# adamnelsonarcher/BB-OCR

Measured on AMD Instinct MI355X. Metric: book-page images/sec end-to-end (detect+recognize) @1280x960, higher is better.
Workload: dtype fp16

## Files before the change

bb-ocr_amd/csrc/common.h:

```cpp
#pragma once
#include <hip/hip_runtime.h>
#include <stdint.h>
#include <atomic>
#include <string>

typedef __attribute__((ext_vector_type(8))) __bf16 bf16x8;
typedef __attribute__((ext_vector_type(8))) short s16x8;
typedef __attribute__((ext_vector_type(4))) float f32x4;
typedef __attribute__((ext_vector_type(4))) unsigned int u32x4;
typedef __attribute__((ext_vector_type(2))) unsigned int u32x2;

static inline uint16_t f32_to_bf16_host(float f) {
    uint32_t u;
    __builtin_memcpy(&u, &f, 4);
    if ((u & 0x7fffffffu) > 0x7f800000u) return (uint16_t)((u >> 16) | 0x40);
    u += 0x7fffu + ((u >> 16) & 1u);
    return (uint16_t)(u >> 16);
}
static inline float bf16_to_f32_host(uint16_t h) {
    uint32_t u = ((uint32_t)h) << 16;
    float f;
    __builtin_memcpy(&f, &u, 4);
    return f;
}
// ... 5 lines not shown
    __bf16 b = (__bf16)f;
    return __builtin_bit_cast(unsigned short, b);
}
typedef __attribute__((ext_vector_type(2))) __bf16 bf16x2_t;
typedef __attribute__((ext_vector_type(2))) float f32x2_t;
__device__ __forceinline__ unsigned int pack_bf16x2(float lo, float hi) {
    const f32x2_t v = {lo, hi};
    return __builtin_bit_cast(unsigned int, __builtin_convertvector(v, bf16x2_t));
}

typedef __attribute__((ext_vector_type(8))) _Float16 f16x8;
typedef __attribute__((ext_vector_type(2))) _Float16 f16x2_t;
static inline uint16_t f32_to_f16_host(float f) {
    const _Float16 h = (_Float16)f;
    uint16_t u;
    __builtin_memcpy(&u, &h, 2);
    return u;
}
static inline float f16_to_f32_host(uint16_t u) {
    _Float16 h;
    __builtin_memcpy(&h, &u, 2);
    return (float)h;
}
static inline uint16_t f32_to_el_host(int el, float f) { return el ? f32_to_f16_host(f) : f32_to_bf16_host(f); }
static inline float el_to_f32_host(int el, uint16_t u) { return el ? f16_to_f32_host(u) : bf16_to_f32_host(u); }

template <int EL> struct El;
template <> struct El<0> {
    typedef bf16x8 v8;
    static __device__ __forceinline__ f32x4 mfma(v8 a, v8 b, f32x4 c) { return __builtin_amdgcn_mfma_f32_16x16x32_bf16(a, b, c, 0, 0, 0); }
    static __device__ __forceinline__ unsigned int pack2(float lo, float hi) { return pack_bf16x2(lo, hi); }
    static __device__ __forceinline__ f32x2_t unpack2(unsigned int q) { return (f32x2_t){__uint_as_float(q << 16), __uint_as_float(q & 0xffff0000u)}; }
    static __device__ __forceinline__ unsigned short from_f32(float f) { return f32_to_bf16_bits(f); }
    static __device__ __forceinline__ float to_f32(unsigned short h) { return bf16_bits_to_f32(h); }
};
template <> struct El<1> {
    typedef f16x8 v8;
    static __device__ __forceinline__ f32x4 mfma(v8 a, v8 b, f32x4 c) { return __builtin_amdgcn_mfma_f32_16x16x32_f16(a, b, c, 0, 0, 0); }
    static __device__ __forceinline__ unsigned int pack2(float lo, float hi) {
        const f32x2_t v = {lo, hi};
        return __builtin_bit_cast(unsigned int, __builtin_convertvector(v, f16x2_t));
    }
    static __device__ __forceinline__ f32x2_t unpack2(unsigned int q) { return __builtin_convertvector(__builtin_bit_cast(f16x2_t, q), f32x2_t); }
    static __device__ __forceinline__ unsigned short from_f32(float f) { return __builtin_bit_cast(unsigned short, (_Float16)f); }
    static __device__ __forceinline__ float to_f32(unsigned short h) { return (float)__builtin_bit_cast(_Float16, h); }
};
__device__ __forceinline__ s16x8 sm16_key(s16x8 x) { return x ^ ((x >> 15) & (short)0x7fff); }

__device__ __forceinline__ int xcd_remap(int bid, int nblk) {
    const int q = nblk >> 3, r = nblk & 7, x = bid & 7, i = bid >> 3;
    return (x < r ? x * (q + 1) : r * (q + 1) + (x - r) * q) + i;
}

#define HIP_TRY(expr)                                                                      \
    do {                                                                                   \
        hipError_t _e = (expr);                                                            \
        if (_e != hipSuccess) {                                                            \
            throw std::string(#expr) + ": " + hipGetErrorString(_e);                       \
        }                                                                                  \
    } while (0)

static constexpr int kMaxDev = 32;
struct LdsOptIn {
    std::atomic<size_t> hw[kMaxDev];
};
static inline hipError_t lds_opt_in(LdsOptIn& st, const void* fn, size_t smem) {
    int d = 0;
    hipError_t e = hipGetDevice(&d);
    if (e != hipSuccess) return e;
    if (d < 0 || d >= kMaxDev) return hipErrorInvalidDevice;
    size_t cur = st.hw[d].load(std::memory_order_acquire);
    if (smem <= cur) return hipSuccess;
    e = hipFuncSetAttribute(fn, hipFuncAttributeMaxDynamicSharedMemorySize, (int)smem);
    if (e != hipSuccess) return e;
    while (cur < smem && !st.hw[d].compare_exchange_weak(cur, smem, std::memory_order_release)) {}
    return hipSuccess;
}
static inline int device_cus() {
    static std::atomic<int> n[kMaxDev];
    int d = 0;
    if (hipGetDevice(&d) != hipSuccess || d < 0 || d >= kMaxDev) return 256;
    int v = n[d].load(std::memory_order_acquire);
    if (v) return v;
    hipDeviceProp_t prop;
    v = (hipGetDeviceProperties(&prop, d) == hipSuccess && prop.multiProcessorCount > 0) ? prop.multiProcessorCount : 256;
    n[d].store(v, std::memory_order_release);
    return v;
}
```

bb-ocr_amd/csrc/conv_mfma.hip:

```cpp
#include "common.h"
#include "kernels.h"
#include <type_traits>
#include <utility>

__device__ __forceinline__ void lds_dma16(const void* gptr, const void* lds) {
    const unsigned la = (unsigned)(size_t)(const __attribute__((address_space(3))) void*)lds;
    asm volatile("s_mov_b32 m0, %1\n\ts_nop 0\n\tglobal_load_lds_dwordx4 %0, off" ::"v"(gptr), "s"(la) : "memory");
}

template <int EL, int MF, bool ADDUP = false>
__device__ __forceinline__ void conv_epilogue(const ConvArgs& a, f32x4 (&acc)[MF][4], int n, int nt, int oy0, int ox0, int wm, int wn, int fpr,
                                              int lane, int BN, int sub = 1, int sph = 0, int spw = 0) {
    const int g = lane >> 4, pl = lane & 15;
    const int cout0 = nt * BN + wn * 64 + g * 8;
    if (a.tail) {
        const float* tw = a.tail;
        const typename El<EL>::v8 w1f = *(const typename El<EL>::v8*)(a.tail_frag + lane * 8);
        float cb[8], b1r[4], w2a[4], w2b[4];
#pragma unroll
        for (int i = 0; i < 8; ++i) cb[i] = a.bias[(g & 1) * 8 + i];
#pragma unroll
        for (int r = 0; r < 4; ++r) { b1r[r] = tw[4 * g + r]; w2a[r] = tw[16 + 4 * g + r]; w2b[r] = tw[32 + 4 * g + r]; }
        const float b20 = tw[48], b21 = tw[49];
#pragma unroll
        for (int f = 0; f < MF; ++f) {
            const int F = wm * MF + f;
            const int fr = F / fpr, fc = F - fr * fpr;
            const int oy = (oy0 + fr) * sub + sph, ox = (ox0 + fc * 16 + pl) * sub + spw;
            u32x4 bb;
#pragma unroll
            for (int j = 0; j < 2; ++j) {
                const float x0 = fmaxf(acc[f][j][0] + cb[j * 4 + 0], 0.f), x1 = fmaxf(acc[f][j][1] + cb[j * 4 + 1], 0.f);
                const float x2 = fmaxf(acc[f][j][2] + cb[j * 4 + 2], 0.f), x3 = fmaxf(acc[f][j][3] + cb[j * 4 + 3], 0.f);
                bb[2 * j] = g < 2 ? El<EL>::pack2(x0, x1) : 0u;
                bb[2 * j + 1] = g < 2 ? El<EL>::pack2(x2, x3) : 0u;
            }
            const f32x4 d = El<EL>::mfma(w1f, __builtin_bit_cast(typename El<EL>::v8, bb), (f32x4){0.f, 0.f, 0.f, 0.f});
            float p0 = 0.f, p1 = 0.f;
#pragma unroll
            for (int r = 0; r < 4; ++r) {
                const float hv = fmaxf(d[r] + b1r[r], 0.f);
                p0 = fmaf(w2a[r], hv, p0);
                p1 = fmaf(w2b[r], hv, p1);
            }
            p0 += __shfl_xor(p0, 16); p1 += __shfl_xor(p1, 16);
            p0 += __shfl_xor(p0, 32); p1 += __shfl_xor(p1, 32);
            if (g == 0 && oy < a.OH && ox < a.OW) *(float2*)((float*)a.out + ((size_t)(n * a.OH + oy) * a.OW + ox) * 2) = make_float2(p0 + b20, p1 + b21);
        }
        return;
    }
    const bool run0 = cout0 < a.cout_store, run1 = cout0 + 32 < a.cout_store;
    if (!run0) return;
    const float sc = a.acc_scale;
    float bs[16];
#pragma unroll
    for (int h = 0; h < 2; ++h)
#pragma unroll
        for (int q = 0; q < 2; ++q) {
            const f32x4 b4 = *(const f32x4*)(a.bias + cout0 + h * 32 + q * 4);
            bs[h * 8 + q * 4 + 0] = b4[0]; bs[h * 8 + q * 4 + 1] = b4[1]; bs[h * 8 + q * 4 + 2] = b4[2]; bs[h * 8 + q * 4 + 3] = b4[3];
        }
// ... 1493 lines not shown
```

bb-ocr_amd/csrc/ctx.h:

```cpp
#pragma once
#include "../../include/bbocr.h"

#include <algorithm>
#include <atomic>
#include <chrono>
#include <condition_variable>
#include <cmath>
#include <cstring>
#include <functional>
#include <map>
#include <memory>
#include <mutex>
#include <string>
#include <thread>
#include <unordered_map>
#include <vector>

#include "boxpost.h"
#include "hostpool.h"
#include "common.h"
#include "kernels.h"


using clk = std::chrono::steady_clock;
// ... 273 lines not shown
};

struct RecChunk {
    int imgW, T, first, n;
    size_t row0;
};

struct RecPart {
    std::vector<CropDesc> descs;
    std::vector<int> order;
    std::vector<RecChunk> chunks;
    size_t rows = 0, cols = 0;
    bool any_warp = false, any_tall = false;
};

struct RecRun {
    std::vector<int> tiles, seqs, seq_k;
    size_t rows = 0;
    int n_results = 0;
};

struct RecEarly {
    bool active = false;
    int pages = 0;
    std::vector<BoxJob> jobs;
    std::vector<int> box_off;
    size_t a_total = 0, w_total = 0;
    RecPart part;
};

constexpr int REC_GAP = 4;
constexpr int REC_STAGES = 8;

template <typename T> inline T* upload(bbocr_ctx* c, const std::vector<T>& v) {
    void* d = nullptr;
    HIPCHK(hipMalloc(&d, v.size() * sizeof(T)));
    c->owned.push_back(d);
    c->owned_bytes.push_back(v.size() * sizeof(T));
    HIPCHK(hipMemcpy(d, v.data(), v.size() * sizeof(T), hipMemcpyHostToDevice));
    return (T*)d;
}

ConvPlan make_plan(int Cin, int Cout, int KH, int KW, int pad, int dil, int el = 0, int bn = 0);
void upload_plan(bbocr_ctx* c, ConvPlan& p, const std::vector<float>& w, const std::vector<float>& b);
void free_weights(bbocr_ctx* c);
size_t weights_blob_bytes(const bbocr_ctx* c);
void weights_export(bbocr_ctx* c, void* dev_dst, size_t bytes);
void weights_import(bbocr_ctx* c, const void* dev_src, size_t bytes);
void load_craft(bbocr_ctx* c, const TensorMap& tm);
void load_crnn(bbocr_ctx* c, const TensorMap& tm);
ConvArgs conv_args(const ConvPlan& p, const Act& a0, const Act* a1 = nullptr, const Act* addup = nullptr);
hipError_t launch_conv_profiled(bbocr_ctx* c, const ConvPlan& p, ConvArgs a, bool may_decline = false);
void run_conv(bbocr_ctx* c, const ConvPlan& p, const Act& a0, bool relu0, const Act* a1, bool relu1, bool relu_out, void* out, int out_cs, int cout_store, bool out_f32, const Act* addup = nullptr);
void prof_collect(bbocr_ctx* c);
Act conv_act(bbocr_ctx* c, const ConvPlan& p, const Act& a0, bool relu0, const Act* a1, bool relu1, bool relu_out, int store);
Act conv_pool_act(bbocr_ctx* c, const ConvPlan& p, const Act& a0, bool relu0, bool relu_out, int store, int mode, bool pool_relu, Act* full, const RgbSource* rgb = nullptr);
Act pool_act(bbocr_ctx* c, const Act& a, int kh, int kw, int sh, int sw, int ph, int pw, bool relu_in);
void craft_up_stage(bbocr_ctx* c, const ConvPlan& py, const ConvPlan& ps, const Act& y, const Act& skip, uint16_t* z, uint16_t* out);
bool craft_up3b_post(bbocr_ctx* c, const Act& u3a, uint16_t* u3b, uint16_t* z);
bool craft_up4(bbocr_ctx* c, const Act& s1, const uint16_t* z, uint16_t* u4b);
void craft_cls_tail(bbocr_ctx* c, const Act& c2, float* heat);
struct ExactConvRow {
    const char* name;
    ConvPlan bbocr_ctx::* plan;
    bool relu_out;
    int store;
    int pool_mode;
    bool pool_relu;
    bool keep_full;
};
int craft_exact_rows();
const ExactConvRow& craft_exact_row(int row);
Act craft_exact_conv(bbocr_ctx* c, int row, const Act& in, Act* full = nullptr);
Act craft_exact_conv1_1(bbocr_ctx* c, const uint8_t* rgb, int nb, int Himg, int Wimg, int H32, int W32);
Act craft_exact_relu(bbocr_ctx* c, const Act& a);
Act craft_exact_upcat(bbocr_ctx* c, const Act& y, const Act& skip);
Act craft_exact_pool5(bbocr_ctx* c, const Act& s4);
void craft_exact_cls_tail(bbocr_ctx* c, const Act& c3, float* heat);
DetDims det_dims(int H, int W, int canvas, double mag);
void detect_impl(bbocr_ctx* c, const uint8_t* rgb, int B, int H, int W, const bbocr_params& p, float* heat, const std::function<void(int, int)>& after_sub = nullptr);
DetPlan det_plan(bbocr_ctx* c, int B, int H, int W, const bbocr_params& p, bool overlapped);
void det_size(bbocr_ctx* c, size_t arena_bytes, size_t resized_bytes);
void det_run(bbocr_ctx* c, const DetPlan& s, const uint8_t* rgb, float* heat, const std::function<void(int, int)>& after_sub = nullptr);
int ccl_cap_comps(int B, int h, int w);
void ccl_size(bbocr_ctx* c, size_t npx, int cap_comps);
void boxes_impl(bbocr_ctx* c, const float* heat, int B, int h, int w, double ratio, const bbocr_params& p, HostBoxes& hb, hipStream_t st);
bbocr_boxlist* export_boxes(const HostBoxes& hb);
void import_boxes(const bbocr_boxlist* bl, HostBoxes& hb);
bool plan_horizontal(const std::array<int, 4>& box, int img, int H, int W, BoxJob& j);
bool plan_free(const std::array<double, 8>& fq, int img, BoxJob& j);
int rec_mode(const bbocr_ctx* c);
void crop_refit_fw(CropDesc& d);
void rec_layout_scratch(std::vector<BoxJob>& jobs, size_t first, size_t& a_total, size_t& w_total);
bool contrast_lut(const unsigned int* hist, size_t npx, double target, uint8_t* lut);
std::vector<int> crop_contrast_luts(bbocr_ctx* c, const CropDesc* descs_dev, std::vector<CropDesc>& descs, double target, std::vector<uint8_t>& luts);
void rec_launch_crops(bbocr_ctx* c, const GrayPages& g, const RecPart& part, const CropDesc* dd, uint16_t* wide, int stage);
void rec_plan_part(const std::vector<BoxJob>& jobs, const std::vector<int>& sel, int res0, size_t row_base, RecPart& part);
const CropDesc* rec_upload_descs(bbocr_ctx* c, const RecPart& part, DevBuf& desc_buf);
uint16_t* rec_wide_image(bbocr_ctx* c, const RecPart& part);
void crnn_features_wide(bbocr_ctx* c, const RecPart& part, const CropDesc* descs, const uint16_t* wide);
Act crnn_stage_shape(const bbocr_ctx* c, const RecPart& part, int stage);
Act crnn_features_stages(bbocr_ctx* c, const RecPart& part, const CropDesc* descs, Act a, int first, int last);
void rec_add_tables(RecRun& run, const RecPart& part, int tile_seqs);
void crnn_sequence(bbocr_ctx* c, size_t rows, size_t rows_pad, const int* tiles_dev, int ntiles, const int* seqs_dev, int nseq, float* logits);
void crnn_seq_xproj(bbocr_ctx* c, int l, const uint16_t* x, size_t rows_pad, void* xp);
void crnn_seq_lin(bbocr_ctx* c, int l, const uint16_t* h, size_t rows_pad, uint16_t* out);
void crnn_seq_pred(bbocr_ctx* c, const uint16_t* x, size_t rows_pad, float* logits);
void rec_seq_tiles(const bbocr_ctx* c, RecRun& run);
enum { CTC_GREEDY = 0, CTC_BEAM_HOST = 1, CTC_BEAM_DEVICE = 2 };
int ctc_route(int beam_width, int C, const int* seqs, int nseq);
void ctc_size(bbocr_ctx* c, size_t rows, int nseq, int cs, int route);
double ctc_decode(const CtcOut& o, const int* idx, int n, std::vector<int>& text);
void rec_early_begin(bbocr_ctx* c, const GrayPages& g, int pages, int B, const HostBoxes& hb, const bbocr_params& p, RecEarly& e);
void recognize_impl(bbocr_ctx* c, const GrayPages& g, int B, const HostBoxes& hb, const bbocr_params& p, std::vector<BoxJob>& jobs, std::vector<int>& box_off, RecEarly* early = nullptr);
bbocr_result* export_result(int B, const std::vector<BoxJob>& jobs, const std::vector<int>& box_off);
void pp_resize(bbocr_ctx* c, const uint8_t* src, int H, int W, uint8_t* dst, int dh, int dw, bool src_bgr = false);
void pp_gauss(bbocr_ctx* c, const uint8_t* src, int H, int W, uint8_t* dst, double sigma);
const uint8_t* pp_fold_lut(bbocr_ctx* c, size_t n, double contrast, double brightness);
void pp_clahe(bbocr_ctx* c, const uint8_t* src, int H, int W, const uint8_t* d_lut, uint8_t* dst, double clip_limit);
void pp_unsharp(bbocr_ctx* c, const uint8_t* src, int H, int W, uint8_t* dst, uint8_t* tmp1, uint8_t* tmp2, float radius, int percent, int threshold);
void preprocess_chain_impl(bbocr_ctx* c, const uint8_t* bgr, int H, int W, const bbocr_preproc_params& q, uint8_t* out, int dh, int dw);
void gaussian_taps_fixed(int n, double sigma, int* k);

inline HostPool& host_pool(bbocr_ctx* c) {
    if (!c->pool) {
        const int want = c->cfg.host_threads > 0 ? c->cfg.host_threads : std::min(16, host_cpu_share());
        c->pool.reset(new HostPool(std::max(1, std::min(want, 64)) - 1));
    }
    return *c->pool;
}

inline bool other_call_in_flight(bbocr_ctx* c) {
    bbocr_ctx* root = c->root;
    std::lock_guard<std::mutex> lk(root->pool_mu);
    if (root != c && root->slot_busy) return true;
    for (bbocr_ctx* s : root->slots)
        if (s != c && s->slot_busy) return true;
    return false;
}

struct EnqLock {
    std::unique_lock<std::mutex> lk;
    explicit EnqLock(bbocr_ctx* c) : lk(c->root->enq_mu) {}
};
constexpr int kMaxSlots = 2;
bbocr_ctx* slot_create(bbocr_ctx* root);
void slot_destroy(bbocr_ctx* s);
void publish_times(const bbocr_ctx* s);
void dist_release(bbocr_ctx* root);

inline void slot_sync(bbocr_ctx* c, hipStream_t st) {
    if (!c->sync_ev) HIPCHK(hipEventCreateWithFlags(&c->sync_ev, hipEventDisableTiming));
    HIPCHK(hipEventRecord(c->sync_ev, st));
    HIPCHK(hipEventSynchronize(c->sync_ev));
}

inline void prof_release(bbocr_ctx* c, const bbocr_ctx::ProfRec& r) { c->prof_pool.push_back(r.e0); c->prof_pool.push_back(r.e1); }

// ... 116 lines not shown
```

bb-ocr_amd/csrc/detector.cpp:

```cpp
#include "ctx.h"

static hipEvent_t prof_event(bbocr_ctx* c) {
    hipEvent_t e;
    if (!c->prof_pool.empty()) { e = c->prof_pool.back(); c->prof_pool.pop_back(); }
    else HIPCHK(hipEventCreate(&e));
    return e;
}

template <typename F> static hipError_t profiled(bbocr_ctx* c, double flops, F&& launch) {
    if (c->profiling == 0 || (c->profiling == 1 && c->prof_group != 0)) return launch();
    bbocr_ctx::ProfRec r{prof_event(c), prof_event(c), flops, c->prof_group};
    HIPCHK(hipEventRecord(r.e0, c->cur));
    const hipError_t e = launch();
    HIPCHK(hipEventRecord(r.e1, c->cur));
    if (e == hipSuccess) c->prof_recs.push_back(r);
    else prof_release(c, r);
    return e;
}

hipError_t launch_conv_profiled(bbocr_ctx* c, const ConvPlan& p, ConvArgs a, bool may_decline) {
    a.zero = c->zero_page;
    const int OH = a.H + 2 * p.pad_h - (p.KH - 1) * p.dil, OW = a.W + 2 * p.pad_w - (p.KW - 1) * p.dil;
    double flops = 2.0 * a.N * OH * OW * (double)p.Cout * (p.split ? p.Cin / 3 : p.Cin) * p.KH * p.KW;
    if (a.c11_w) flops += 2.0 * a.N * a.H * a.W * 64.0 * 27.0;
    if (a.tail) flops += 2.0 * a.N * OH * OW * (16.0 * 16.0 + 16.0 * 2.0);
    if (a.post_w) flops += 2.0 * a.N * OH * OW * 64.0 * 64.0;
    const hipError_t e = profiled(c, flops, [&] { return launch_conv(p, a, c->cur); });
    if (may_decline && e == hipErrorNotSupported) return e;
    HIPCHK(e);
    return hipSuccess;
}

ConvArgs conv_args(const ConvPlan& p, const Act& a0, const Act* a1, const Act* addup) {
    ConvArgs a{};
    a.in0 = a0.p; a.C0 = a0.C; a.in0_cs = a0.C;
    a.N = a0.N; a.H = a0.H; a.W = a0.W;
    if (p.split) {
        if (a1 || (a0.C & 63)) fail(BBOCR_ERR_INTERNAL, "split-fp16 conv: one pair tensor with a multiple of 32 logical channels expected");
        a.in1 = a0.p; a.C1 = a0.C / 2; a.in1_cs = a0.C;
    } else if (a1) {
        a.in1 = a1->p; a.C1 = a1->C; a.in1_cs = a1->C;
    }
    if (addup) { a.addup = addup->p; a.up_H = a0.H; a.up_W = a0.W; a.up_cs = addup->C; }
    return a;
}

void run_conv(bbocr_ctx* c, const ConvPlan& p, const Act& a0, bool relu0, const Act* a1, bool relu1, bool relu_out, void* out,
                     int out_cs, int cout_store, bool out_f32, const Act* addup) {
    if (c->arena.dry) return;
    ConvArgs a = conv_args(p, a0, a1, addup);
    a.relu_in0 = relu0; a.relu_in1 = p.split ? relu0 : relu1; a.relu_out = relu_out; a.out_f32 = out_f32;
    a.out = out; a.out_cs = out_cs; a.cout_store = cout_store;
    if (p.split && !out_f32) a.split_off = cout_store;
    (void)launch_conv_profiled(c, p, a);
}

void prof_collect(bbocr_ctx* c) {
    bbocr_ctx* root = c->root;
    std::lock_guard<std::mutex> lk(root->pool_mu);
    for (auto& r : c->prof_recs) {
        float ms = 0.f;
        if (hipEventElapsedTime(&ms, r.e0, r.e1) == hipSuccess) {
            root->prof_ms[r.group] += ms;
            root->prof_flops[r.group] += r.flops;
            root->prof_launches[r.group] += 1;
        }
        prof_release(c, r);
    }
    c->prof_recs.clear();
}

static Act arena_act(bbocr_ctx* c, int N, int H, int W, int C) { return Act{c->arena.alloc<uint16_t>((size_t)N * H * W * C), N, H, W, C}; }

Act conv_act(bbocr_ctx* c, const ConvPlan& p, const Act& a0, bool relu0, const Act* a1, bool relu1, bool relu_out, int store) {
    const int OH = a0.H + 2 * p.pad_h - (p.KH - 1) * p.dil, OW = a0.W + 2 * p.pad_w - (p.KW - 1) * p.dil;
    const int cs = p.split ? 2 * store : store;
    Act o = arena_act(c, a0.N, OH, OW, cs);
    run_conv(c, p, a0, relu0, a1, relu1, relu_out, o.p, cs, store, false);
    return o;
}

Act conv_pool_act(bbocr_ctx* c, const ConvPlan& p, const Act& a0, bool relu0, bool relu_out, int store, int mode, bool pool_relu,
                         Act* full, const RgbSource* rgb) {
// ... 387 lines not shown
```

bb-ocr_amd/csrc/kernels.h:

```cpp
#pragma once
#include <hip/hip_runtime.h>
#include <stdint.h>
#include <vector>

struct ConvArgs {
    const uint16_t* in0;
    const uint16_t* in1;
    const uint16_t* wpk;
    const float* bias;
    void* out;
    int C0, C1;
    int in0_cs, in1_cs;
    int N, H, W, OH, OW;
    int KH, KW, pad_h, pad_w, dil;
    int TH, TW, tiles_x, tiles_y, ntiles_n;
    int PH, PW, NP;
    int relu_in0, relu_in1, relu_out, out_f32;
    int out_cs, cout_store;
    int nchunks, ntaps;
    int pool_mode, pool_relu, store_full, pool_cs;
    void* pool_out;
    const uint16_t* aux_w;
    const float* tail;
    const uint16_t* tail_frag;
// ... 80 lines not shown
hipError_t launch_pair_relu(const uint16_t* in, uint16_t* out, size_t npix, int C, hipStream_t s);
hipError_t launch_pair_maxpool3x3s1(const uint16_t* in, uint16_t* out, int N, int H, int W, int C, hipStream_t s);
hipError_t launch_pair_upcat(const uint16_t* y, int yh, int yw, int Cy, const uint16_t* skip, int Cs, uint16_t* out, int N, int H, int W, hipStream_t s);
hipError_t launch_pair_cls_tail(const uint16_t* in , const float* w1 , const float* tail , float* heat,
                                size_t npix, hipStream_t s);

struct CclOut {
    int root, left, top, right, bottom, area, row_off, img;
};
hipError_t launch_ccl(const float* heat, int N, int h, int w, float low_text, float link_thr, double text_thr, int* label, int* stat,
                      int* slot, CclOut* comps, int* rowext, int* counters, int cap_comps, int cap_rows, hipStream_t s);

struct CropDesc {
    int img;
    int sx0, sy0, sw, sh;
    int rw, rh;
    int fw;
    int imgW;
    int slot;
    int warp;
    int warp_off;
    int a_off;
    int lut_off;
    int pad_;
    int rot;
    double Minv[9];
};
struct CropPage {
    long long off;
    long long pitch;
    int H, W;
};
hipError_t launch_crops(const uint8_t* gray, int H, int W, const CropDesc* descs_dev, int first, int count, int imgW, int any_warp,
                        int any_tall, uint8_t* wscratch, uint8_t* scratch, uint8_t* hscratch, const uint8_t* luts, uint16_t* out_bucket,
                        int stage_mask, hipStream_t s, int wide_row_stride = 0, int gap = 0, int mode = 0,
                        const CropPage* pages = nullptr);
enum { REC_BF16 = 0, REC_F16 = 1, REC_SPLIT = 2 };
constexpr float SPLIT_LO_SCALE = 2048.f;
hipError_t launch_crop_hist(const uint8_t* scratch, const CropDesc* descs_dev, int first, int count, unsigned int* hist, hipStream_t s);
hipError_t launch_crnn_conv0(const uint16_t* in, const float* w , const float* b, uint16_t* out, int n, int W, int mode, hipStream_t s,
                             const uint16_t* afrag = nullptr );
void pack_crnn_conv0_mfma(const float* w_tap_major , uint16_t* out , int el);
hipError_t launch_crnn_zero_gaps(uint16_t* t, const CropDesc* descs_dev, int first, int count, int H, int Wl, int C, int shift, hipStream_t s);
hipError_t launch_rowmean3_gather(const uint16_t* in, int Wc, int C, const CropDesc* descs_dev, int first, int count, uint16_t* out, int mode,
                                  hipStream_t s);
hipError_t launch_lstm(const void* xproj, const uint16_t* whh_pk, uint16_t* out, const int* tiles_dev, int ntiles, int mode, float acc_scale,
                       hipStream_t s);
int lstm_tile_seqs(int mode);
size_t lstm_whh_packed_elems();
void pack_lstm_whh8(const float* whh_fwd, const float* whh_bwd, uint16_t* out, int el);
size_t lstm_whh_split_packed_elems();
float pack_lstm_whh_split(const float* whh_fwd, const float* whh_bwd, uint16_t* out);
int lstm8_xproj_channel(int dir, int gate, int unit);
size_t q8_packed_bytes(int N, int K);
void pack_q8_weights(const int8_t* q , int N, int K, int8_t* out);
void pack_q8_whh(const int8_t* q_fwd, const int8_t* q_bwd , int8_t* out );
hipError_t launch_q8_quantize(const void* x, int src_pair, int K, size_t rows, size_t rows_pad, const int* seqs_dev, int nseq, float* rowp, int8_t* a8,
                              uint8_t* codes, float* segp, hipStream_t s);
hipError_t launch_q8_gemm(const int8_t* a8, size_t rows_pad, int K, const int8_t* wpk, int N, const float* rowp, const float* wscale, const float* bias,
                          float* out, int ldo, hipStream_t s);
constexpr int LSTM_Q8_SEQS = 16;
hipError_t launch_lstm_q8(const float* G, const int8_t* whh_pk, const float* whh_scale, const float* bhh, float* out, const int* seqs_dev,
                          const int* tiles_dev, int ntiles, float* c_out, uint8_t* hcodes, float* hparams, hipStream_t s);
struct CtcOut { int len; int cnt; float prod; int pad; };
hipError_t launch_ctc(const float* logits, size_t rows, int C, int cs, const int* seqs_dev, int nseq, int* idx_tmp, float* pmax_tmp,
                      int* out_idx, CtcOut* out, hipStream_t s, const unsigned int* ignore = nullptr, float* probs_out = nullptr);
void ctc_beam_search_host(const float* mat, int T, int C, int cs, int beam_width, std::vector<int>& text);
class HostPool;
void ctc_beam_search_batch(const float* probs, const int* seqs, int nseq, int C, int cs, int beam_width, std::vector<std::vector<int>>& texts,
                           HostPool* pool = nullptr);
constexpr size_t kCtcBeamLdsLimit = 65536;
size_t ctc_beam_lds_bytes(int beam_width, int C, int max_T);
bool ctc_beam_on_device(int beam_width, int C, int max_T);
hipError_t launch_ctc_beam(const float* probs, size_t rows, int C, int cs, const int* seqs_dev, int nseq, int max_T, int beam_width, int* out_text,
                           int* out_len, hipStream_t s);

int pp_resize_tile_rows(int H, int W, int dh, int dw);
hipError_t launch_pp_resize_cubic(const uint8_t* src, int H, int W, uint8_t* dst, int dh, int dw, const int* x0, const double* wx, const long long* nx,
                                  const int* y0, const double* wy, const long long* ny, unsigned long long KX, unsigned long long KY, hipStream_t s, int src_bgr = 0);
hipError_t launch_pp_gauss3(const uint8_t* src, int H, int W, uint8_t* dst, int k0, int k1, int k2, unsigned long long* sum, hipStream_t s);
hipError_t launch_pp_clahe_hist(const uint8_t* src, int H, int W, const uint8_t* lut, int tw, int th, int tx, int ty, unsigned int* hist,
                                hipStream_t s);
hipError_t launch_pp_clahe_apply(const uint8_t* src, int H, int W, const uint8_t* lut, const uint8_t* tile_luts, int tw, int th, int tx, int ty,
                                 uint8_t* dst, hipStream_t s);
hipError_t launch_pp_box_pass(const uint8_t* src, uint8_t* dst, int H, int W, int vertical, int r, unsigned int ww, unsigned int fw, hipStream_t s);
hipError_t launch_pp_fold_lut(const unsigned long long* sum, unsigned long long n, float contrast, float brightness, uint8_t* lut, hipStream_t s);
hipError_t launch_pp_clahe_luts(const unsigned int* hist, int tiles, int clip, float lut_scale, uint8_t* tile_luts, hipStream_t s);
hipError_t launch_pp_lut(const uint8_t* src, uint8_t* dst, const uint8_t* lut, size_t total, hipStream_t s);
bool pp_unsharp_fused_ok(int H, int W, int r, const uint8_t* a, const uint8_t* b, const uint8_t* c);
hipError_t launch_pp_unsharp_fused(const uint8_t* in, uint8_t* tmp, uint8_t* dst, int H, int W, unsigned int ww, unsigned int fw, int percent,
                                   int threshold, hipStream_t s);
hipError_t launch_pp_unsharp(const uint8_t* in, const uint8_t* blur, uint8_t* dst, size_t total, int percent, int threshold, hipStream_t s);

constexpr int AC_BOX = 35, AC_BOX_R = 17, AC_MEAN_C = 10;
constexpr int AC_GAU = 31, AC_GAU_R = 15, AC_GAU_C = 5;
struct AcTaps { int k[AC_GAU]; };
hipError_t launch_ac_gray_blur(const uint8_t* src, int H, int W, size_t pitch, int channels, uint8_t* dst, hipStream_t s);
hipError_t launch_ac_cues(const uint8_t* e, int H, int W, const AcTaps& taps, uint16_t* rbox, uint16_t* rgau, uint8_t* part, uint8_t* grad,
                          unsigned int* hist, int* thr, hipStream_t s);
hipError_t launch_ac_pack(const uint8_t* e, const uint8_t* part, const uint8_t* grad, const int* thr, int H, int W, int WW, uint32_t* bits, hipStream_t s);
hipError_t launch_ac_rect(const uint32_t* src, uint32_t* tmp, uint32_t* dst, int H, int W, int WW, int rx, int ry, int erode, const uint32_t* or_with,
                          hipStream_t s);
hipError_t launch_ac_components(const uint32_t* bits, int H, int W, int WW, int* label, uint8_t* flag, int* count, int cap, int* boxes, hipStream_t s);
hipError_t launch_ac_unpack(const uint32_t* bits, const int* label, int H, int W, int WW, uint8_t* dst, hipStream_t s);

enum : int { PAGE_GRAY = 0, PAGE_BGR = 1, PAGE_RGB = 2, PAGE_YCC4 = 3, PAGE_YCC3 = 4 };
// ... 135 lines not shown
```

bb-ocr_amd/csrc/recognizer.cpp:

```cpp
#include "ctx.h"

void crop_refit_fw(CropDesc& d) {
    const int cw = (int)std::ceil(64 * ((double)d.rw / (double)d.rh));
    d.fw = cw > d.imgW ? d.imgW : cw;
}

static bool plan_sizes(CropDesc& d, int width, int height) {
    double ratio = (double)width / (double)height;
    if (ratio < 1.0) {
        ratio = 1.0 / ratio;
        d.rw = 64; d.rh = (int)(64 * ratio);
    } else {
        d.rw = (int)(64 * ratio); d.rh = 64;
    }
    if ((int)(64 * ratio) == 0) return false;
    d.imgW = (int)std::ceil(std::max(ratio, 1.0)) * 64;
    crop_refit_fw(d);
    return d.rw > 0 && d.rh > 0 && d.fw > 0;
}

bool plan_horizontal(const std::array<int, 4>& box, int img, int H, int W, BoxJob& j) {
    const int x_min = std::max(0, box[0]), x_max = std::min(box[1], W), y_min = std::max(0, box[2]), y_max = std::min(box[3], H);
    const int width = x_max - x_min, height = y_max - y_min;
    if (width <= 0 || height <= 0) return false;
// ... 86 lines not shown
    c->seq_rowp.ensure(rows_pad * 16);
    int8_t* a8 = (int8_t*)c->seq_q8.p;
    float* rowp = (float*)c->seq_rowp.p;
    auto qlinear = [&](const void* x, int pair, int K, const bbocr_ctx::Q8Layer& L, int N, float* out) {
        HIPCHK(launch_q8_quantize(x, pair, K, rows, rows_pad, seqs_dev, nseq, rowp, a8, nullptr, nullptr, c->cur));
        HIPCHK(launch_q8_gemm(a8, rows_pad, K, L.w, N, rowp, L.scale, L.bias, out, N, c->cur));
    };
    const void* cur = c->seq_v.p;
    for (int l = 0; l < 2; ++l) {
        qlinear(cur, l == 0, 256, c->q_ih[l], 2048, (float*)c->seq_xp.p);
        HIPCHK(launch_lstm_q8((const float*)c->seq_xp.p, c->q_hh[l].w, c->q_hh[l].scale, c->q_hh[l].bias, (float*)c->seq_h.p, seqs_dev, tiles_dev, ntiles,
                              nullptr, nullptr, nullptr, c->cur));
        float* dst = (float*)(l == 0 ? c->seq_lin.p : c->seq_v.p);
        qlinear(c->seq_h.p, 0, 512, c->q_lin[l], 256, dst);
        cur = dst;
    }
    qlinear(cur, 0, 256, c->q_pred, 112, logits);
}

void rec_seq_tiles(const bbocr_ctx* c, RecRun& run) {
    if (!rec_quant(c)) return;
    run.tiles.clear();
    const int nseq = (int)(run.seqs.size() / 2);
    for (int s0 = 0; s0 < nseq; s0 += LSTM_Q8_SEQS) {
        const int n = std::min(LSTM_Q8_SEQS, nseq - s0);
        int tmax = 0;
        for (int i = 0; i < n; ++i) tmax = std::max(tmax, run.seqs[2 * (s0 + i) + 1]);
        const int t[4] = {s0, n, tmax, 0};
        run.tiles.insert(run.tiles.end(), t, t + 4);
    }
}

void crnn_sequence(bbocr_ctx* c, size_t rows, size_t rows_pad, const int* tiles_dev, int ntiles, const int* seqs_dev, int nseq, float* logits) {
    c->prof_group = 1;
    c->arena.dry = false;
    if (rec_quant(c)) { crnn_sequence_q8(c, rows, rows_pad, tiles_dev, ntiles, seqs_dev, nseq, logits); return; }
    const bool sp = rec_split(c);
    const int m = rec_mul(c);
    c->seq_xp.ensure(rows_pad * 2048 * (sp ? 4 : 2));
    c->seq_h.ensure(rows_pad * 512 * 2 * m);
    c->seq_lin.ensure(rows_pad * 256 * 2 * m);
    const uint16_t* cur = (const uint16_t*)c->seq_v.p;
    for (int l = 0; l < 2; ++l) {
        crnn_seq_xproj(c, l, cur, rows_pad, c->seq_xp.p);
        HIPCHK(launch_lstm(c->seq_xp.p, c->whh[l], (uint16_t*)c->seq_h.p, tiles_dev, ntiles, rec_mode(c), c->whh_scale[l], c->cur));
        uint16_t* dst = (uint16_t*)(l == 0 ? c->seq_lin.p : c->seq_v.p);
        crnn_seq_lin(c, l, (const uint16_t*)c->seq_h.p, rows_pad, dst);
        cur = dst;
    }
    crnn_seq_pred(c, cur, rows_pad, logits);
}

static Act seq_rows(const bbocr_ctx* c, const uint16_t* p, size_t rows_pad, int C) { return Act{(uint16_t*)p, 1, (int)(rows_pad / 256), 256, C * rec_mul(c)}; }
void crnn_seq_xproj(bbocr_ctx* c, int l, const uint16_t* x, size_t rows_pad, void* xp) {
    run_conv(c, c->xproj[l], seq_rows(c, x, rows_pad, 256), false, nullptr, false, false, xp, 2048, 2048, rec_split(c));
}
void crnn_seq_lin(bbocr_ctx* c, int l, const uint16_t* h, size_t rows_pad, uint16_t* out) {
    run_conv(c, c->lin[l], seq_rows(c, h, rows_pad, 512), false, nullptr, false, false, out, 256 * rec_mul(c), 256, false);
}
void crnn_seq_pred(bbocr_ctx* c, const uint16_t* x, size_t rows_pad, float* logits) {
    run_conv(c, c->pred, seq_rows(c, x, rows_pad, 256), false, nullptr, false, false, logits, 112, 112, true);
}

static size_t rec_max_rows(const bbocr_ctx* c) { return c->cfg.rec_max_cols > 0 ? (size_t)std::max(64, c->cfg.rec_max_cols / 4) : (size_t)1500000; }

void rec_plan_part(const std::vector<BoxJob>& jobs, const std::vector<int>& sel, int res0, size_t row_base, RecPart& part) {
    std::map<int, std::vector<int>> buckets;
    for (size_t k = 0; k < sel.size(); ++k) buckets[jobs[sel[k]].d.imgW].push_back((int)k);
    size_t rows = row_base, cols = 0;
    for (auto& kv : buckets) {
        const int imgW = kv.first, T = imgW / 4 - 1;
        RecChunk ch{imgW, T, (int)part.descs.size(), (int)kv.second.size(), rows};
        for (int i = 0; i < ch.n; ++i) {
            const int k = kv.second[i];
            CropDesc d = jobs[sel[k]].d;
            if (cols > 0x7ff00000u) fail(BBOCR_ERR_OVERFLOW, "recogniser pass wider than 2^31 columns");
            d.slot = (int)cols;
            d.pad_ = (int)(rows + (size_t)i * T);
            cols += (size_t)imgW + REC_GAP;
            part.any_warp |= d.warp != 0;
            part.any_tall |= !(d.fw == d.rw && d.rh == 64);
            part.descs.push_back(d);
            part.order.push_back(res0 + k);
        }
        rows += (size_t)ch.n * T;
        part.chunks.push_back(ch);
    }
    part.rows = rows - row_base;
    part.cols = cols;
}

const CropDesc* rec_upload_descs(bbocr_ctx* c, const RecPart& part, DevBuf& desc_buf) {
    const size_t bytes = part.descs.size() * sizeof(CropDesc);
    desc_buf.ensure(bytes);
    PinBuf& pin = (&desc_buf == &c->crop_desc2) ? c->desc_pin2 : c->desc_pin;
    pin.ensure(bytes);
    memcpy(pin.p, part.descs.data(), bytes);
    HIPCHK(hipMemcpyAsync(desc_buf.p, pin.p, bytes, hipMemcpyHostToDevice, c->stream));
    return (const CropDesc*)desc_buf.p;
}

uint16_t* rec_wide_image(bbocr_ctx* c, const RecPart& part) {
    c->arena.begin(true);
    (void)c->arena.alloc<uint16_t>((size_t)64 * part.cols);
    crnn_features_wide(c, part, nullptr, nullptr);
    c->arena.buf.ensure(c->arena.off);
    c->arena.begin(false);
    return c->arena.alloc<uint16_t>((size_t)64 * part.cols);
// ... 449 lines not shown
```

Before: 975.1.

## Add dedicated weight-stationary persistent kernel for LSTM input projection

Adds a specialized GEMM kernel for the 256->2048 LSTM input projection. Each block keeps its 256-column weight slice in registers and streams 64-row slots of activations through a 4-deep LDS ring filled by direct global-to-LDS DMA, with counted vmcnt waits to overlap loads, MFMA and stores. It replaces the generic conv path when split mode is off and falls back to it otherwise. This trades generality and register pressure for removing repeated weight loads and pipeline overhead.

```diff
diff --git a/bb-ocr_amd/csrc/common.h b/bb-ocr_amd/csrc/common.h
--- a/bb-ocr_amd/csrc/common.h
+++ b/bb-ocr_amd/csrc/common.h
@@ -81,7 +81,12 @@
     return (x < r ? x * (q + 1) : r * (q + 1) + (x - r) * q) + i;
 }
 
-#define HIP_TRY(expr)                                                                      \
+__device__ __forceinline__ void lds_dma16(const void* gptr, const void* lds) {
+    const unsigned la = (unsigned)(size_t)(const __attribute__((address_space(3))) void*)lds;
+    asm volatile("s_mov_b32 m0, %1\n\ts_nop 0\n\tglobal_load_lds_dwordx4 %0, off" ::"v"(gptr), "s"(la) : "memory");
+}
+
+#define HIP_TRY(expr)                                                                     \
     do {                                                                                   \
         hipError_t _e = (expr);                                                            \
         if (_e != hipSuccess) {                                                            \
diff --git a/bb-ocr_amd/csrc/conv_mfma.hip b/bb-ocr_amd/csrc/conv_mfma.hip
--- a/bb-ocr_amd/csrc/conv_mfma.hip
+++ b/bb-ocr_amd/csrc/conv_mfma.hip
@@ -2,11 +2,6 @@
 #include "kernels.h"
 #include <type_traits>
 #include <utility>
-
-__device__ __forceinline__ void lds_dma16(const void* gptr, const void* lds) {
-    const unsigned la = (unsigned)(size_t)(const __attribute__((address_space(3))) void*)lds;
-    asm volatile("s_mov_b32 m0, %1\n\ts_nop 0\n\tglobal_load_lds_dwordx4 %0, off" ::"v"(gptr), "s"(la) : "memory");
-}
 
 template <int EL, int MF, bool ADDUP = false>
 __device__ __forceinline__ void conv_epilogue(const ConvArgs& a, f32x4 (&acc)[MF][4], int n, int nt, int oy0, int ox0, int wm, int wn, int fpr,
diff --git a/bb-ocr_amd/csrc/ctx.h b/bb-ocr_amd/csrc/ctx.h
--- a/bb-ocr_amd/csrc/ctx.h
+++ b/bb-ocr_amd/csrc/ctx.h
@@ -349,6 +349,7 @@
 ConvArgs conv_args(const ConvPlan& p, const Act& a0, const Act* a1 = nullptr, const Act* addup = nullptr);
 hipError_t launch_conv_profiled(bbocr_ctx* c, const ConvPlan& p, ConvArgs a, bool may_decline = false);
 void run_conv(bbocr_ctx* c, const ConvPlan& p, const Act& a0, bool relu0, const Act* a1, bool relu1, bool relu_out, void* out, int out_cs, int cout_store, bool out_f32, const Act* addup = nullptr);
+hipError_t launch_seq_proj_profiled(bbocr_ctx* c, const ConvPlan& p, const uint16_t* x, size_t rows_pad, uint16_t* out);
 void prof_collect(bbocr_ctx* c);
 Act conv_act(bbocr_ctx* c, const ConvPlan& p, const Act& a0, bool relu0, const Act* a1, bool relu1, bool relu_out, int store);
 Act conv_pool_act(bbocr_ctx* c, const ConvPlan& p, const Act& a0, bool relu0, bool relu_out, int store, int mode, bool pool_relu, Act* full, const RgbSource* rgb = nullptr);
@@ -401,6 +402,7 @@
 void rec_add_tables(RecRun& run, const RecPart& part, int tile_seqs);
 void crnn_sequence(bbocr_ctx* c, size_t rows, size_t rows_pad, const int* tiles_dev, int ntiles, const int* seqs_dev, int nseq, float* logits);
 void crnn_seq_xproj(bbocr_ctx* c, int l, const uint16_t* x, size_t rows_pad, void* xp);
+void crnn_seq_xproj_conv(bbocr_ctx* c, int l, const uint16_t* x, size_t rows_pad, void* xp);
 void crnn_seq_lin(bbocr_ctx* c, int l, const uint16_t* h, size_t rows_pad, uint16_t* out);
 void crnn_seq_pred(bbocr_ctx* c, const uint16_t* x, size_t rows_pad, float* logits);
 void rec_seq_tiles(const bbocr_ctx* c, RecRun& run);
diff --git a/bb-ocr_amd/csrc/detector.cpp b/bb-ocr_amd/csrc/detector.cpp
--- a/bb-ocr_amd/csrc/detector.cpp
+++ b/bb-ocr_amd/csrc/detector.cpp
@@ -29,6 +29,13 @@
     if (may_decline && e == hipErrorNotSupported) return e;
     HIPCHK(e);
     return hipSuccess;
+}
+
+hipError_t launch_seq_proj_profiled(bbocr_ctx* c, const ConvPlan& p, const uint16_t* x, size_t rows_pad, uint16_t* out) {
+    const double flops = 2.0 * (double)rows_pad * (double)p.Cout * p.Cin;
+    const hipError_t e = profiled(c, flops, [&] { return launch_seq_proj(p, x, rows_pad, out, c->cur); });
+    if (e != hipErrorNotSupported) HIPCHK(e);
+    return e;
 }
 
 ConvArgs conv_args(const ConvPlan& p, const Act& a0, const Act* a1, const Act* addup) {
diff --git a/bb-ocr_amd/csrc/kernels.h b/bb-ocr_amd/csrc/kernels.h
--- a/bb-ocr_amd/csrc/kernels.h
+++ b/bb-ocr_amd/csrc/kernels.h
@@ -156,6 +156,9 @@
 size_t lstm_whh_split_packed_elems();
 float pack_lstm_whh_split(const float* whh_fwd, const float* whh_bwd, uint16_t* out);
 int lstm8_xproj_channel(int dir, int gate, int unit);
+struct SeqProjPlan { int grid, chunks, ring; long long nslots, chunk_slots; };
+SeqProjPlan seq_proj_plan(size_t rows_pad, int ncu);
+hipError_t launch_seq_proj(const ConvPlan& p, const uint16_t* x, size_t rows_pad, uint16_t* out, hipStream_t s);
 size_t q8_packed_bytes(int N, int K);
 void pack_q8_weights(const int8_t* q , int N, int K, int8_t* out);
 void pack_q8_whh(const int8_t* q_fwd, const int8_t* q_bwd , int8_t* out );
diff --git a/bb-ocr_amd/csrc/recognizer.cpp b/bb-ocr_amd/csrc/recognizer.cpp
--- a/bb-ocr_amd/csrc/recognizer.cpp
+++ b/bb-ocr_amd/csrc/recognizer.cpp
@@ -162,8 +162,15 @@
 }
 
 static Act seq_rows(const bbocr_ctx* c, const uint16_t* p, size_t rows_pad, int C) { return Act{(uint16_t*)p, 1, (int)(rows_pad / 256), 256, C * rec_mul(c)}; }
+void crnn_seq_xproj_conv(bbocr_ctx* c, int l, const uint16_t* x, size_t rows_pad, void* xp) {
+    run_conv(c, c->xproj[l], seq_rows(c, x, rows_pad, 256), false, nullptr, false, false, xp, 2048, 2048, rec_split(c));
+}
 void crnn_seq_xproj(bbocr_ctx* c, int l, const uint16_t* x, size_t rows_pad, void* xp) {
-    run_conv(c, c->xproj[l], seq_rows(c, x, rows_pad, 256), false, nullptr, false, false, xp, 2048, 2048, rec_split(c));
+    if (!rec_split(c)) {
+        if (c->arena.dry) return;
+        if (launch_seq_proj_profiled(c, c->xproj[l], x, rows_pad, (uint16_t*)xp) == hipSuccess) return;
+    }
+    crnn_seq_xproj_conv(c, l, x, rows_pad, xp);
 }
 void crnn_seq_lin(bbocr_ctx* c, int l, const uint16_t* h, size_t rows_pad, uint16_t* out) {
     run_conv(c, c->lin[l], seq_rows(c, h, rows_pad, 512), false, nullptr, false, false, out, 256 * rec_mul(c), 256, false);
diff --git a/bb-ocr_amd/csrc/seq_proj.hip b/bb-ocr_amd/csrc/seq_proj.hip
--- /dev/null
+++ b/bb-ocr_amd/csrc/seq_proj.hip
@@ -0,0 +1,130 @@
+#include "common.h"
+#include "kernels.h"
+
+namespace {
+constexpr int SP_K = 256, SP_N = 2048;
+constexpr int SP_WAVES = 8, SP_COLS = SP_WAVES * 64, SP_CG = SP_N / SP_COLS;
+constexpr int SP_RING = 4, SP_SLOT_ROWS = 64, SP_SLOT = SP_SLOT_ROWS * SP_K * 2;
+constexpr int SP_DMAS = SP_SLOT / 1024 / SP_WAVES;
+constexpr int SP_STORES = (SP_SLOT_ROWS / 16) * 2;
+constexpr size_t SP_LDS = (size_t)SP_RING * SP_SLOT;
+static_assert(SP_DMAS * SP_WAVES * 1024 == SP_SLOT && SP_DMAS == SP_SLOT_ROWS / 16 && SP_WAVES == SP_K / 32, "wave w fetches k-step w of the slot's four 16-row blocks");
+static_assert((SP_RING - 1) * SP_STORES + (SP_RING - 2) * SP_DMAS < 64, "the counted wait must fit vmcnt's 6 bits");
+
+template <int EL>
+__global__ void __launch_bounds__(SP_WAVES * 64, 2) seq_proj_kernel(const uint16_t* __restrict__ x, const uint16_t* __restrict__ wpk, const float* __restrict__ bias,
+                                                                    uint16_t* __restrict__ out, float acc_scale, int nslots, int chunk_slots) {
+    typedef typename El<EL>::v8 v8;
+    extern __shared__ __attribute__((aligned(16))) unsigned char smem[];
+    const int lane = threadIdx.x & 63;
+    const int wave = __builtin_amdgcn_readfirstlane(threadIdx.x >> 6);
+    const int bid = xcd_remap(blockIdx.x, gridDim.x);
+    const int cg = bid % SP_CG, chunk = bid / SP_CG;
+    const int s0 = chunk * chunk_slots;
+    const int n = nslots - s0 < chunk_slots ? nslots - s0 : chunk_slots;
+    if (n <= 0) return;
+    const int nt = cg * 2 + (wave >> 2), wn = wave & 3;
+    const int g = lane >> 4, pl = lane & 15;
+    const int cout0 = nt * 256 + wn * 64 + g * 8;
+
+    typedef const __attribute__((address_space(1))) v8* gfrag_ptr;
+    const gfrag_ptr wg = (gfrag_ptr)((const v8*)wpk + ((size_t)nt * 8 * 16 + wn * 4) * 64 + lane);
+    v8 w[8][4];
+#pragma unroll
+    for (int ks = 0; ks < 8; ++ks)
+#pragma unroll
+        for (int j = 0; j < 4; ++j) w[ks][j] = wg[(ks * 16 + j) * 64];
+    f32x4 bs[4];
+#pragma unroll
+    for (int j = 0; j < 4; ++j) bs[j] = *(const __attribute__((address_space(1))) f32x4*)(bias + cout0 + (j >> 1) * 32 + (j & 1) * 4);
+
+    const uint16_t* src = x + ((size_t)s0 * SP_SLOT_ROWS + (lane >> 2)) * SP_K + wave * 32 + ((lane & 3) ^ (((lane >> 4) & 1) * 2)) * 8;
+    auto issue = [&](int s, int ring) {
+        unsigned char* sb = smem + ring * SP_SLOT + wave * 4096;
+#pragma unroll
+        for (int i = 0; i < SP_DMAS; ++i) lds_dma16(src + ((size_t)s * SP_SLOT_ROWS + i * 16) * SP_K, sb + i * 1024);
+    };
+#pragma unroll
+    for (int i = 0; i < SP_RING - 1; ++i)
+        if (i < n) issue(i, i);
+    asm volatile("s_waitcnt vmcnt(0) lgkmcnt(0)\n\ts_barrier" ::: "memory");
+#pragma unroll
+    for (int ks = 0; ks < 8; ++ks)
+#pragma unroll
+        for (int j = 0; j < 4; ++j) asm volatile("" : "+v"(w[ks][j]));
+#pragma unroll
+    for (int j = 0; j < 4; ++j) asm volatile("" : "+v"(bs[j]));
+
+    const int lane_p_off = pl * 64 + (g ^ (((pl >> 2) & 1) * 2)) * 16;
+    uint16_t* op = out + ((size_t)s0 * SP_SLOT_ROWS + (pl & 7)) * SP_N + cout0 + (pl >> 3) * 32;
+    int ring = 0;
+    for (int s = 0; s < n; ++s) {
+        const bool ahead = s + SP_RING - 1 < n;
+        if (ahead) {
+            int r2 = ring + SP_RING - 1;
+            if (r2 >= SP_RING) r2 -= SP_RING;
+            issue(s + SP_RING - 1, r2);
+        }
+        const unsigned char* sb = smem + ring * SP_SLOT + lane_p_off;
+#pragma unroll
+        for (int b = 0; b < SP_SLOT_ROWS / 16; ++b) {
+            v8 bq[8];
+#pragma unroll
+            for (int ks = 0; ks < 8; ++ks) bq[ks] = *(const v8*)(sb + ks * 4096 + b * 1024);
+            f32x4 acc[4];
+#pragma unroll
+            for (int j = 0; j < 4; ++j) acc[j] = (f32x4){0.f, 0.f, 0.f, 0.f};
+#pragma unroll
+            for (int ks = 0; ks < 8; ++ks)
+#pragma unroll
+                for (int j = 0; j < 4; ++j) acc[j] = El<EL>::mfma(w[ks][j], bq[ks], acc[j]);
+            float v[16];
+#pragma unroll
+            for (int j = 0; j < 4; ++j)
+#pragma unroll
+                for (int r = 0; r < 4; ++r) v[j * 4 + r] = fmaf(acc[j][r], acc_scale, bs[j][r]);
+            const u32x4 lo = {El<EL>::pack2(v[0], v[1]), El<EL>::pack2(v[2], v[3]), El<EL>::pack2(v[4], v[5]), El<EL>::pack2(v[6], v[7])};
+            const u32x4 hi = {El<EL>::pack2(v[8], v[9]), El<EL>::pack2(v[10], v[11]), El<EL>::pack2(v[12], v[13]), El<EL>::pack2(v[14], v[15])};
+            u32x4 dA, dB;
+#pragma unroll
+            for (int i = 0; i < 4; ++i) {
+                dA[i] = (unsigned)__builtin_amdgcn_update_dpp((int)lo[i], (int)hi[i], 0x118 , 0xF, 0xC, false);
+                dB[i] = (unsigned)__builtin_amdgcn_update_dpp((int)hi[i], (int)lo[i], 0x108 , 0xF, 0x3, false);
+            }
+            *(u32x4*)op = dA;
+            *(u32x4*)(op + 8 * SP_N) = dB;
+            op += 16 * SP_N;
+        }
+        if (ahead) asm volatile("s_waitcnt vmcnt(%0) lgkmcnt(0)\n\ts_barrier" ::"n"((SP_RING - 1) * SP_STORES + (SP_RING - 2) * SP_DMAS) : "memory");
+        else asm volatile("s_waitcnt vmcnt(%0) lgkmcnt(0)\n\ts_barrier" ::"n"((SP_RING - 1) * SP_STORES) : "memory");
+        ring = ring + 1 == SP_RING ? 0 : ring + 1;
+    }
+}
+}
+
+SeqProjPlan seq_proj_plan(size_t rows_pad, int ncu) {
+    SeqProjPlan p{};
+    int chunks = ncu / SP_CG / 8 * 8;
+    if (chunks < 8) chunks = 8;
+    const size_t nslots = rows_pad / SP_SLOT_ROWS;
+    p.chunks = chunks;
+    p.ring = SP_RING;
+    p.grid = chunks * SP_CG;
+    p.nslots = (long long)nslots;
+    p.chunk_slots = (long long)((nslots + chunks - 1) / chunks);
+    return p;
+}
+
+hipError_t launch_seq_proj(const ConvPlan& p, const uint16_t* x, size_t rows_pad, uint16_t* out, hipStream_t s) {
+    if (p.KH != 1 || p.KW != 1 || p.Cin != SP_K || p.Cin_pad != SP_K || p.Cout != SP_N || p.Cout_pad != SP_N || p.BN != 256 || p.split || !p.d_w || !p.d_b)
+        return hipErrorNotSupported;
+    if (!x || !out || rows_pad == 0 || rows_pad % 256 != 0) return hipErrorNotSupported;
+    const SeqProjPlan g = seq_proj_plan(rows_pad, device_cus());
+    if (g.nslots + g.chunks > 0x7fffffffLL) return hipErrorNotSupported;
+    static LdsOptIn attr[2];
+    const void* k = p.el ? (const void*)seq_proj_kernel<1> : (const void*)seq_proj_kernel<0>;
+    if (hipError_t e = lds_opt_in(attr[p.el ? 1 : 0], k, SP_LDS); e != hipSuccess) return e;
+    if (p.el) hipLaunchKernelGGL(seq_proj_kernel<1>, dim3(g.grid), dim3(SP_WAVES * 64), SP_LDS, s, x, p.d_w, p.d_b, out, p.acc_scale, (int)g.nslots, (int)g.chunk_slots);
+    else hipLaunchKernelGGL(seq_proj_kernel<0>, dim3(g.grid), dim3(SP_WAVES * 64), SP_LDS, s, x, p.d_w, p.d_b, out, p.acc_scale, (int)g.nslots, (int)g.chunk_slots);
+    return hipGetLastError();
+}
```

New measurement: 991.7 (median of 6 runs). +1.7%, better.
